# ActiveVisionLab/CrossScore

Measured on AMD Instinct MI355X. Metric: query-images/sec at 518x518, 5 ref views, bs=8; score-map MAE vs ref, higher is better.
Workload: dtype fp16

## Files before the change

### crossscore_amd/build.py

```python
from __future__ import annotations

import os
import subprocess
import sys

HERE = os.path.dirname(os.path.abspath(__file__))
CSRC = os.path.join(HERE, "csrc")
LIB = os.path.join(HERE, "libcrossscore_hip.so")
SOURCES = ["api.hip", "gemm.hip", "gemm256.hip", "attention.hip", "elementwise.hip", "preprocess.hip", "panel.hip", "panel4.hip", "patch.hip", "rowln.hip"]


EXTRA_FLAGS = {"panel.hip": ["-fno-slp-vectorize"], "panel4.hip": ["-fno-slp-vectorize"]}


def _hipcc() -> str:
    for c in (os.environ.get("HIPCC"), "/opt/rocm/bin/hipcc", "hipcc"):
        if c and (os.path.isabs(c) and os.path.exists(c) or not os.path.isabs(c)):
            return c
    return "hipcc"


def needs_build() -> bool:
    if not os.path.exists(LIB):
        return True
    t = os.path.getmtime(LIB)
    deps = [os.path.join(CSRC, f) for f in os.listdir(CSRC)] + [os.path.join(os.path.dirname(HERE), "include", "crossscore_hip.h")]
    return any(os.path.getmtime(d) > t for d in deps)


def build(force: bool = False, verbose: bool = True) -> str:
    if not force and not needs_build():
        return LIB
    objs = []
    procs = []
    os.makedirs(os.path.join(HERE, "build"), exist_ok=True)
    for s in SOURCES:
        o = os.path.join(HERE, "build", s.replace(".hip", ".o"))
        objs.append(o)
        cmd = [_hipcc(), "--offload-arch=gfx950", "-O3", "-std=c++17", "-fPIC", "-Wno-unused-value"] + EXTRA_FLAGS.get(s, []) + ["-c", os.path.join(CSRC, s), "-o", o]
        procs.append((cmd, subprocess.Popen(cmd, stdout=subprocess.PIPE, stderr=subprocess.STDOUT, text=True)))
    for cmd, p in procs:
        out, _ = p.communicate()
        if p.returncode != 0:
            raise RuntimeError("hipcc failed: " + " ".join(cmd) + "\n" + out)
        if verbose and out.strip():
            print(out, file=sys.stderr)
    cmd = [_hipcc(), "--offload-arch=gfx950", "-shared", "-fPIC", "-o", LIB] + objs
    r = subprocess.run(cmd, stdout=subprocess.PIPE, stderr=subprocess.STDOUT, text=True)
    if r.returncode != 0:
        raise RuntimeError("link failed: " + r.stdout)
    return LIB


if __name__ == "__main__":
    print(build(force="--force" in sys.argv))
```

### crossscore_amd/csrc/attention.hip

```cpp
#include "cs_common.h"
#include <atomic>
#include <math.h>

#ifdef CS_ATTN_STAMP
__device__ unsigned long long g_attn_dbg[64 * 4 * 8];
#define CS_TS(k) do { __builtin_amdgcn_sched_barrier(0); const unsigned long long now_ = __builtin_amdgcn_s_memtime(); \
    ph[k] += now_ - tlast; tlast = now_; __builtin_amdgcn_sched_barrier(0); } while (0)
#else
#define CS_TS(k) do { } while (0)
#endif

namespace {

template <int DH>
struct AttnCfg {
  static constexpr int KS = DH / 16;
  static constexpr int DT = (DH + 31) / 32;
  static constexpr int CH = DH / 8;
  static constexpr int KROW = DH * 2 + 16;
  static constexpr int VROW = (DH <= 16) ? 64 : (DH <= 96 ? 192 : (DH <= 128 ? 320 : 448));
  static_assert(VROW >= DT * 64 && (VROW / 4) % 32 == 16, "V row pitch");
  static constexpr int KTILE = 64 * KROW;
  static constexpr int VTILE = 64 * VROW;
  static constexpr int STAGE = KTILE + VTILE;
  static constexpr int NIT = (64 * CH + 255) / 256;
};

template <int DH, bool BF>
__global__ __launch_bounds__(256, DH > 128 ? 1 : 2) void cs_attn_kernel(CsAttnParams p) {
  using Cfg = AttnCfg<DH>;
  constexpr int KS = Cfg::KS, DT = Cfg::DT, CH = Cfg::CH, NIT = Cfg::NIT;
  extern __shared__ __attribute__((aligned(16))) char smem[];
  const int tid = threadIdx.x;
  const int lane = tid & 63;
  const int wv = __builtin_amdgcn_readfirstlane(tid >> 6);
  const int r = lane & 31;
  const int hh = lane >> 5;
  const int QB = (p.Lq + 127) / 128;
  const int xcd = blockIdx.x & 7, jj = blockIdx.x >> 3;
  const int gi = jj / QB, qb = jj - gi * QB;
  const int grp = gi * 8 + xcd;
  if (grp >= p.heads * p.nbatch) return;
  const int head = grp % p.heads;
  const int bat = grp / p.heads;
  const int q0 = qb * 128 + wv * 32;

  const h16_t* Qb = p.Q + (size_t)bat * p.q_bs + head * DH;
  const h16_t* Kb = p.K + (size_t)bat * p.k_bs + head * DH;
  const h16_t* Vb = p.V + (size_t)bat * p.v_bs + head * DH;

  h16x8_t qf[KS];
  {
    int qr = q0 + r;
    qr = qr < p.Lq ? qr : p.Lq - 1;
    const h16_t* qp = Qb + (size_t)qr * p.ldq + 8 * hh;
#pragma unroll
    for (int s = 0; s < KS; ++s) qf[s] = *reinterpret_cast<const h16x8_t*>(qp + 16 * s);
  }

  constexpr bool kFullLast = (64 * CH) % 256 == 0;
  int skey[NIT], sch[NIT];
#pragma unroll
  for (int it = 0; it < NIT; ++it) {
    const int c = tid + it * 256;
    skey[it] = c / CH;
    sch[it] = c - skey[it] * CH;
  }
  uint4 kreg[NIT], vreg[NIT];
#pragma unroll
  for (int it = 0; it < NIT; ++it) { kreg[it] = make_uint4(0, 0, 0, 0); vreg[it] = make_uint4(0, 0, 0, 0); }
  unsigned kgo[NIT], vgo[NIT];
#pragma unroll
  for (int it = 0; it < NIT; ++it) {
    kgo[it] = ((unsigned)skey[it] * (unsigned)p.ldk + (unsigned)sch[it] * 8u) * 2u;
    vgo[it] = ((unsigned)skey[it] * (unsigned)p.ldv + (unsigned)sch[it] * 8u) * 2u;
  }
  const unsigned k_bytes = (unsigned)(((size_t)(p.Lk - 1) * p.ldk + DH) * 2), v_bytes = (unsigned)(((size_t)(p.Lk - 1) * p.ldv + DH) * 2);
#define CS_ATTN_LOAD_TILE(T)                                                                       \
  {                                                                                                \
    const unsigned ks_ = (unsigned)(T) * 64u * (unsigned)p.ldk * 2u, vs_ = (unsigned)(T) * 64u * (unsigned)p.ldv * 2u; \
    const __amdgpu_buffer_rsrc_t k_rs = __builtin_amdgcn_make_buffer_rsrc(                         \
        const_cast<char*>(reinterpret_cast<const char*>(Kb)) + ks_, 0, (int)(k_bytes - ks_), 0x00020000); \
    const __amdgpu_buffer_rsrc_t v_rs = __builtin_amdgcn_make_buffer_rsrc(                         \
        const_cast<char*>(reinterpret_cast<const char*>(Vb)) + vs_, 0, (int)(v_bytes - vs_), 0x00020000); \
    _Pragma("unroll") for (int it = 0; it < NIT; ++it) {                                           \
      if (kFullLast || it + 1 < NIT || tid + it * 256 < 64 * CH) {                                 \
        kreg[it] = __builtin_bit_cast(uint4, __builtin_amdgcn_raw_buffer_load_b128(k_rs, kgo[it], 0, 0)); \
        vreg[it] = __builtin_bit_cast(uint4, __builtin_amdgcn_raw_buffer_load_b128(v_rs, vgo[it], 0, 0)); \
      }                                                                                            \
    }                                                                                              \
  }
#define CS_ATTN_WRITE_TILE(BUF)                                                                    \
  _Pragma("unroll") for (int it = 0; it < NIT; ++it) {                                             \
    if (kFullLast || it + 1 < NIT || tid + it * 256 < 64 * CH) {                                   \
      char* kb_ = smem + (BUF) * Cfg::STAGE;                                                       \
      *reinterpret_cast<uint4*>(kb_ + skey[it] * Cfg::KROW + sch[it] * 16) = kreg[it];             \
      *reinterpret_cast<uint4*>(kb_ + Cfg::KTILE + skey[it] * Cfg::VROW + sch[it] * 16) = vreg[it]; \
    }                                                                                              \
  }

  f32x16_t ot[DT];
#pragma unroll
  for (int d = 0; d < DT; ++d)
#pragma unroll
    for (int e = 0; e < 16; ++e) ot[d][e] = 0.f;
  constexpr float kTau = 8.0f;
  float m_run = 0.f;
  float l_run = 0.f;
  f32x16_t negm;
#pragma unroll
  for (int e = 0; e < 16; ++e) negm[e] = 0.f;
  {
    const float sc = p.scale_log2e;
    if (sc != 1.0f) {
#pragma unroll
      for (int s = 0; s < KS; ++s)
#pragma unroll
        for (int j = 0; j < 8; ++j) {
          const _Float16 e = qf[s][j];
          qf[s][j] = __builtin_bit_cast(_Float16, f2o<BF>(o2f<BF>(__builtin_bit_cast(h16_t, e)) * sc));
        }
    }
  }

  const int koff = r * Cfg::KROW + hh * 16;
  const int li = lane & 15, lg = (lane >> 4) & 1;
  const int voff = (4 * hh + (li >> 2)) * Cfg::VROW + (16 * lg + 4 * (li & 3)) * 2;

  const int nt = (p.Lk + 63) / 64;
  CS_ATTN_LOAD_TILE(0)
  CS_ATTN_WRITE_TILE(0)
  __syncthreads();
#ifdef CS_ATTN_STAMP
  unsigned long long ph[5] = {0, 0, 0, 0, 0};
  const unsigned long long tbegin = __builtin_amdgcn_s_memtime(), rbegin = __builtin_amdgcn_s_memrealtime();
  unsigned long long tlast = tbegin;
#endif
  for (int t = 0; t < nt; ++t) {
    if (t + 1 < nt) { CS_ATTN_LOAD_TILE(t + 1) }
    const char* kb = smem + (t & 1) * Cfg::STAGE;
    const char* vb = kb + Cfg::KTILE;

    f32x16_t st[2];
    float ps0 = 0.f, ps1 = 0.f;
    h16x8_t pf[2][2];
    auto scores = [&]() {
#pragma unroll
      for (int k2 = 0; k2 < 2; ++k2) {
#pragma unroll
        for (int s = 0; s < KS; ++s) {
          h16x8_t kf = *reinterpret_cast<const h16x8_t*>(kb + koff + k2 * 32 * Cfg::KROW + s * 32);
          st[k2] = mfma_32x32x16<BF>(kf, qf[s], s == 0 ? negm : st[k2]);
        }
      }
      if (t == nt - 1 && (p.Lk & 63)) {
        const int kbase = t * 64 + 4 * hh;
#pragma unroll
        for (int k2 = 0; k2 < 2; ++k2)
#pragma unroll
          for (int e = 0; e < 16; ++e) {
            const int key = kbase + k2 * 32 + (e & 3) + 8 * (e >> 2);
            if (key >= p.Lk) st[k2][e] = -INFINITY;
          }
      }
    };
    auto row_max = [&]() {
      float tm = st[0][0];
#pragma unroll
      for (int e = 1; e < 16; ++e) tm = fmaxf(tm, st[0][e]);
#pragma unroll
      for (int e = 0; e < 16; ++e) tm = fmaxf(tm, st[1][e]);
      return fmaxf(tm, __shfl_xor(tm, 32, 64));
    };
    auto move_reference = [&](float delta, bool first) {
      const float alpha = first ? 1.0f : __builtin_amdgcn_exp2f(-delta);
      m_run += delta;
#pragma unroll
      for (int e = 0; e < 16; ++e) negm[e] = -m_run;
      asm volatile("" : "+v"(negm));
#pragma unroll
      for (int k2 = 0; k2 < 2; ++k2)
#pragma unroll
        for (int e = 0; e < 16; ++e) st[k2][e] -= delta;
      l_run *= alpha;
#pragma unroll
      for (int d = 0; d < DT; ++d)
#pragma unroll
        for (int e = 0; e < 16; ++e) ot[d][e] *= alpha;
    };
    auto exp_pack = [&]() {
      ps0 = 0.f; ps1 = 0.f;
#pragma unroll
      for (int k2 = 0; k2 < 2; ++k2)
#pragma unroll
        for (int s2 = 0; s2 < 2; ++s2) {
#pragma unroll
          for (int j = 0; j < 8; j += 2) {
            const float pa = __builtin_amdgcn_exp2f(st[k2][8 * s2 + j]);
            const float pb = __builtin_amdgcn_exp2f(st[k2][8 * s2 + j + 1]);
            ps0 += pa;
            ps1 += pb;
            pf[k2][s2][j] = __builtin_bit_cast(_Float16, f2o<BF>(pa));
            pf[k2][s2][j + 1] = __builtin_bit_cast(_Float16, f2o<BF>(pb));
          }
        }
    };
    scores();
    const float tmax = row_max();
    CS_TS(0);
    if (t == 0 || __builtin_amdgcn_ballot_w64(tmax > kTau) != 0) move_reference(t == 0 ? tmax : fmaxf(tmax, 0.f), t == 0);
    exp_pack();
    l_run += ps0 + ps1;
    CS_TS(1);

#pragma unroll
    for (int k2 = 0; k2 < 2; ++k2)
#pragma unroll
      for (int s2 = 0; s2 < 2; ++s2) {
        const char* vrow = vb + voff + (k2 * 32 + 16 * s2) * Cfg::VROW;
#pragma unroll
        for (int d = 0; d < DT; ++d) {
          short4_t lo = __builtin_amdgcn_ds_read_tr16_b64_v4i16(
              (__attribute__((address_space(3))) short4_t*)(vrow + d * 64));
          short4_t hi = __builtin_amdgcn_ds_read_tr16_b64_v4i16(
              (__attribute__((address_space(3))) short4_t*)(vrow + 8 * Cfg::VROW + d * 64));
          short8_t vf8 = __builtin_shufflevector(lo, hi, 0, 1, 2, 3, 4, 5, 6, 7);
          ot[d] = mfma_32x32x16<BF>(__builtin_bit_cast(h16x8_t, vf8), pf[k2][s2], ot[d]);
        }
      }

    CS_TS(2);
    if (t + 1 < nt) { CS_ATTN_WRITE_TILE((t + 1) & 1) }
    CS_TS(3);
    __syncthreads();
    CS_TS(4);
  }
#ifdef CS_ATTN_STAMP
  if (blockIdx.x % 50 == 0 && blockIdx.x / 50 < 64 && lane == 0) {
    unsigned long long* d = g_attn_dbg + (blockIdx.x / 50 * 4 + wv) * 8;
    for (int k = 0; k < 5; ++k) d[k] = ph[k];
    d[5] = rbegin;
    d[6] = __builtin_amdgcn_s_memtime() - tbegin;
    d[7] = __builtin_amdgcn_s_memrealtime() - rbegin;
  }
#endif

  const float l_tot = l_run + __shfl_xor(l_run, 32, 64);
  const float inv = 1.0f / l_tot;
  const int q = q0 + r;
  if (q < p.Lq) {
    h16_t* op = p.O + (size_t)bat * p.o_bs + (size_t)q * p.ldo + head * DH;
#pragma unroll
    for (int d = 0; d < DT; ++d)
#pragma unroll
      for (int g4 = 0; g4 < 4; ++g4) {
        const int dd = d * 32 + 8 * g4 + 4 * hh;
        if (dd < DH) {
          const float v0 = ot[d][4 * g4 + 0] * inv, v1 = ot[d][4 * g4 + 1] * inv, v2 = ot[d][4 * g4 + 2] * inv, v3 = ot[d][4 * g4 + 3] * inv;
          uint2 o;
          o.x = pack_o16x2<BF>(v0, v1);
          o.y = pack_o16x2<BF>(v2, v3);
          *reinterpret_cast<uint2*>(op + dd) = o;
        }
      }
    if (p.lse && hh == 0) p.lse[((size_t)bat * p.heads + head) * p.Lq + q] = m_run + log2f(l_tot);
  }
}

template <int DH, bool BF>
hipError_t launch(CsAttnParams p, int batch, hipStream_t stream) {
  p.nbatch = batch;
  const int groups = p.heads * batch;
  dim3 grid(((groups + 7) / 8) * 8 * ((p.Lq + 127) / 128));
  const int lds = 2 * AttnCfg<DH>::STAGE + 64;
  if (lds > 48 * 1024) {
    static std::atomic<bool> attr_done[16];
    int dev = 0;
    if (hipGetDevice(&dev) != hipSuccess || dev < 0 || dev >= 16) return hipErrorInvalidDevice;
    if (!attr_done[dev]) {
      hipError_t e = hipFuncSetAttribute(reinterpret_cast<const void*>(cs_attn_kernel<DH, BF>), hipFuncAttributeMaxDynamicSharedMemorySize, lds);
      if (e != hipSuccess) return e;
      attr_done[dev] = true;
    }
  }
  hipLaunchKernelGGL((cs_attn_kernel<DH, BF>), grid, dim3(256), lds, stream, p);
  return hipGetLastError();
}

}

#ifdef CS_ATTN_STAMP
extern "C" int cs_attn_debug_read(unsigned long long* dst) { return (int)hipMemcpyFromSymbol(dst, HIP_SYMBOL(g_attn_dbg), sizeof(g_attn_dbg)); }
#endif

extern "C" const char* cs_attn_check(const CsAttnParams* p, int dh, int batch) {
  if (dh != 16 && dh != 48 && dh != 64 && dh != 96 && dh != 128 && dh != 192) return "attention: head dim must be 16, 48, 64, 96, 128 or 192";
  if (p->Lq <= 0 || p->Lk <= 0 || p->heads <= 0 || batch <= 0) return "attention: empty shape";
  if ((long long)batch * p->heads * ((p->Lq + 127) / 128) > (1ll << 30)) return "attention: grid too large";
  if (p->ldq % 8 || p->ldk % 8 || p->ldv % 8 || p->ldo % 4) return "attention: row strides must keep 16-byte rows";
  if (p->q_bs % 8 || p->k_bs % 8 || p->v_bs % 8 || p->o_bs % 4) return "attention: batch strides must keep 16-byte rows";
  if (!p->Q || !p->K || !p->V || !p->O) return "attention: null operand";
  if ((long long)p->Lk * p->ldk >= (1ll << 30) || (long long)p->Lk * p->ldv >= (1ll << 30)) return "attention: Lk * row stride must stay below 2^30 elements (32-bit tile offsets)";
  return nullptr;
}

extern "C" hipError_t cs_attn_launch(const CsAttnParams* p, int dh, int batch, hipStream_t stream) {
  switch (dh) {
    case 16: return p->bf16 ? launch<16, true>(*p, batch, stream) : launch<16, false>(*p, batch, stream);
    case 48: return p->bf16 ? launch<48, true>(*p, batch, stream) : launch<48, false>(*p, batch, stream);
    case 64: return p->bf16 ? launch<64, true>(*p, batch, stream) : launch<64, false>(*p, batch, stream);
    case 96: return p->bf16 ? launch<96, true>(*p, batch, stream) : launch<96, false>(*p, batch, stream);
    case 128: return p->bf16 ? launch<128, true>(*p, batch, stream) : launch<128, false>(*p, batch, stream);
    case 192: return p->bf16 ? launch<192, true>(*p, batch, stream) : launch<192, false>(*p, batch, stream);
  }
  return hipErrorInvalidValue;
}
```

Before: 1325.

## Add 16x16x32 MFMA attention path for head dims 48/64 with full/tail tile split

For head dims 48 and 64, the attention kernel now uses 16x16x32 MFMA tiles with two 16-row query sub-tiles per wave. It also uses tighter K/V LDS row pitches, which lets the launch bound allow 3 blocks per CU. This removes the padding waste the 32x32 tiles incurred at small head dims and cuts LDS footprint. Both the new path and the generic path now specialise full tiles versus the ragged last tile, skip dead query waves and half-empty key blocks, and compile with SLP vectorisation off. The risks are more code, higher register pressure from two accumulator sets, and possible correctness issues in the masking/zero-padding for DH=48.

```diff
diff --git a/crossscore_amd/build.py b/crossscore_amd/build.py
--- a/crossscore_amd/build.py
+++ b/crossscore_amd/build.py
@@ -10,7 +10,7 @@
 SOURCES = ["api.hip", "gemm.hip", "gemm256.hip", "attention.hip", "elementwise.hip", "preprocess.hip", "panel.hip", "panel4.hip", "patch.hip", "rowln.hip"]
 
 
-EXTRA_FLAGS = {"panel.hip": ["-fno-slp-vectorize"], "panel4.hip": ["-fno-slp-vectorize"]}
+EXTRA_FLAGS = {"panel.hip": ["-fno-slp-vectorize"], "panel4.hip": ["-fno-slp-vectorize"], "attention.hip": ["-fno-slp-vectorize"]}
 
 
 def _hipcc() -> str:
diff --git a/crossscore_amd/csrc/attention.hip b/crossscore_amd/csrc/attention.hip
--- a/crossscore_amd/csrc/attention.hip
+++ b/crossscore_amd/csrc/attention.hip
@@ -1,6 +1,7 @@
 #include "cs_common.h"
 #include <atomic>
 #include <math.h>
+#include <type_traits>
 
 #ifdef CS_ATTN_STAMP
 __device__ unsigned long long g_attn_dbg[64 * 4 * 8];
@@ -14,12 +15,16 @@
 
 template <int DH>
 struct AttnCfg {
+  static constexpr bool T16 = DH == 48 || DH == 64;
   static constexpr int KS = DH / 16;
   static constexpr int DT = (DH + 31) / 32;
+  static constexpr int KS2 = (DH + 31) / 32;
+  static constexpr int DT16 = DH / 16;
   static constexpr int CH = DH / 8;
-  static constexpr int KROW = DH * 2 + 16;
-  static constexpr int VROW = (DH <= 16) ? 64 : (DH <= 96 ? 192 : (DH <= 128 ? 320 : 448));
-  static_assert(VROW >= DT * 64 && (VROW / 4) % 32 == 16, "V row pitch");
+  static constexpr int KROW = T16 ? 160 : DH * 2 + 16;
+  static constexpr int VROW = T16 ? (DH == 64 ? 160 : 96) : (DH <= 16) ? 64 : (DH <= 96 ? 192 : (DH <= 128 ? 320 : 448));
+  static_assert(T16 ? (VROW >= DH * 2 && (VROW / 4) % 16 == 8 && KROW >= KS2 * 64 && (KROW / 16) % 4 == 2)
+                    : (VROW >= DT * 64 && (VROW / 4) % 32 == 16), "K / V row pitch");
   static constexpr int KTILE = 64 * KROW;
   static constexpr int VTILE = 64 * VROW;
   static constexpr int STAGE = KTILE + VTILE;
@@ -27,7 +32,7 @@
 };
 
 template <int DH, bool BF>
-__global__ __launch_bounds__(256, DH > 128 ? 1 : 2) void cs_attn_kernel(CsAttnParams p) {
+__global__ __launch_bounds__(256, DH > 128 ? 1 : (AttnCfg<DH>::T16 ? 3 : 2)) void cs_attn_kernel(CsAttnParams p) {
   using Cfg = AttnCfg<DH>;
   constexpr int KS = Cfg::KS, DT = Cfg::DT, CH = Cfg::CH, NIT = Cfg::NIT;
   extern __shared__ __attribute__((aligned(16))) char smem[];
@@ -49,15 +54,6 @@
   const h16_t* Kb = p.K + (size_t)bat * p.k_bs + head * DH;
   const h16_t* Vb = p.V + (size_t)bat * p.v_bs + head * DH;
 
-  h16x8_t qf[KS];
-  {
-    int qr = q0 + r;
-    qr = qr < p.Lq ? qr : p.Lq - 1;
-    const h16_t* qp = Qb + (size_t)qr * p.ldq + 8 * hh;
-#pragma unroll
-    for (int s = 0; s < KS; ++s) qf[s] = *reinterpret_cast<const h16x8_t*>(qp + 16 * s);
-  }
-
   constexpr bool kFullLast = (64 * CH) % 256 == 0;
   int skey[NIT], sch[NIT];
 #pragma unroll
@@ -99,6 +95,227 @@
     }                                                                                              \
   }
 
+  if constexpr (Cfg::T16) {
+    constexpr int KS2 = Cfg::KS2, DT16 = Cfg::DT16;
+    const int li = lane & 15, g = lane >> 4;
+    const int nqt = __builtin_amdgcn_readfirstlane(q0 >= p.Lq ? 0 : (q0 + 16 >= p.Lq ? 1 : 2));
+    if constexpr (DH == 48) {
+      const int zrow = (tid >> 1) & 63;
+      *reinterpret_cast<uint4*>(smem + (tid >> 7) * Cfg::STAGE + zrow * Cfg::KROW + 96 + 16 * (tid & 1)) = make_uint4(0, 0, 0, 0);
+    }
+    h16x8_t qf[2][KS2];
+#pragma unroll
+    for (int qt = 0; qt < 2; ++qt) {
+      int qr = q0 + 16 * qt + li;
+      qr = qr < p.Lq ? qr : p.Lq - 1;
+      const h16_t* qp = Qb + (size_t)qr * p.ldq + 8 * g;
+#pragma unroll
+      for (int s = 0; s < KS2; ++s) {
+#pragma unroll
+        for (int j = 0; j < 8; ++j) qf[qt][s][j] = (_Float16)0.f;
+        if (32 * s + 32 <= DH || 32 * s + 8 * g < DH) qf[qt][s] = *reinterpret_cast<const h16x8_t*>(qp + 32 * s);
+      }
+    }
+    {
+      const float sc = p.scale_log2e;
+      if (sc != 1.0f) {
+#pragma unroll
+        for (int qt = 0; qt < 2; ++qt)
+#pragma unroll
+          for (int s = 0; s < KS2; ++s)
+#pragma unroll
+            for (int j = 0; j < 8; ++j) {
+              const _Float16 e = qf[qt][s][j];
+              qf[qt][s][j] = __builtin_bit_cast(_Float16, f2o<BF>(o2f<BF>(__builtin_bit_cast(h16_t, e)) * sc));
+            }
+      }
+    }
+    f32x4_t ot[2][DT16];
+#pragma unroll
+    for (int qt = 0; qt < 2; ++qt)
+#pragma unroll
+      for (int d = 0; d < DT16; ++d)
+#pragma unroll
+        for (int e = 0; e < 4; ++e) ot[qt][d][e] = 0.f;
+    constexpr float kTau = 8.0f;
+    float m_run[2] = {0.f, 0.f};
+    float l_run[2] = {0.f, 0.f};
+    f32x4_t negm[2];
+#pragma unroll
+    for (int qt = 0; qt < 2; ++qt)
+#pragma unroll
+      for (int e = 0; e < 4; ++e) negm[qt][e] = 0.f;
+
+    const int koff = li * Cfg::KROW + g * 16;
+    const int voff = (4 * g + (li >> 2)) * Cfg::VROW + (li & 3) * 8;
+
+    const int nt = (p.Lk + 63) / 64;
+    CS_ATTN_LOAD_TILE(0)
+    CS_ATTN_WRITE_TILE(0)
+    __syncthreads();
+#ifdef CS_ATTN_STAMP
+    unsigned long long ph[5] = {0, 0, 0, 0, 0};
+    const unsigned long long tbegin = __builtin_amdgcn_s_memtime(), rbegin = __builtin_amdgcn_s_memrealtime();
+    unsigned long long tlast = tbegin;
+#endif
+    auto tile = [&](auto full_c, const int t, const int nkt) __attribute__((always_inline)) {
+      constexpr bool FULL = decltype(full_c)::value;
+      const char* kb = smem + (t & 1) * Cfg::STAGE;
+      const char* vb = kb + Cfg::KTILE;
+      f32x4_t st[2][4];
+      h16x8_t pf[2][2];
+      float tm[2] = {-INFINITY, -INFINITY};
+#pragma unroll
+      for (int kt = 0; kt < 4; ++kt) {
+        if (FULL || kt < nkt) {
+          if (!FULL) __builtin_amdgcn_sched_barrier(0);
+#pragma unroll
+          for (int s = 0; s < KS2; ++s) {
+            const h16x8_t kf = *reinterpret_cast<const h16x8_t*>(kb + koff + kt * 16 * Cfg::KROW + s * 64);
+#pragma unroll
+            for (int qt = 0; qt < 2; ++qt)
+              if (FULL || qt < nqt) st[qt][kt] = mfma_16x16x32<BF>(kf, qf[qt][s], s == 0 ? negm[qt] : st[qt][kt]);
+          }
+#pragma unroll
+          for (int qt = 0; qt < 2; ++qt)
+            if (FULL || qt < nqt) {
+              if (!FULL) {
+                const int key = t * 64 + kt * 16 + 4 * g;
+#pragma unroll
+                for (int j = 0; j < 4; ++j)
+                  if (key + j >= p.Lk) st[qt][kt][j] = -INFINITY;
+              }
+#pragma unroll
+              for (int j = 0; j < 4; ++j) tm[qt] = fmaxf(tm[qt], st[qt][kt][j]);
+            }
+        }
+      }
+      CS_TS(0);
+      if (t == 0 || __builtin_amdgcn_ballot_w64(fmaxf(tm[0], tm[1]) > kTau) != 0) {
+#pragma unroll
+        for (int qt = 0; qt < 2; ++qt)
+          if (FULL || qt < nqt) {
+            float rm = fmaxf(tm[qt], __shfl_xor(tm[qt], 16, 64));
+            rm = fmaxf(rm, __shfl_xor(rm, 32, 64));
+            const float delta = t == 0 ? rm : fmaxf(rm, 0.f);
+            const float alpha = t == 0 ? 1.0f : __builtin_amdgcn_exp2f(-delta);
+            m_run[qt] += delta;
+#pragma unroll
+            for (int e = 0; e < 4; ++e) negm[qt][e] = -m_run[qt];
+            asm volatile("" : "+v"(negm[qt]));
+#pragma unroll
+            for (int kt = 0; kt < 4; ++kt)
+              if (FULL || kt < nkt)
+#pragma unroll
+                for (int j = 0; j < 4; ++j) st[qt][kt][j] -= delta;
+            l_run[qt] *= alpha;
+#pragma unroll
+            for (int d = 0; d < DT16; ++d)
+#pragma unroll
+              for (int e = 0; e < 4; ++e) ot[qt][d][e] *= alpha;
+          }
+      }
+      if (!FULL) __builtin_amdgcn_sched_barrier(0);
+#pragma unroll
+      for (int qt = 0; qt < 2; ++qt)
+        if (FULL || qt < nqt) {
+          float ps0 = 0.f, ps1 = 0.f;
+#pragma unroll
+          for (int kt = 0; kt < 4; ++kt) {
+            if (FULL || kt < nkt) {
+#pragma unroll
+              for (int j = 0; j < 4; j += 2) {
+                const float pa = __builtin_amdgcn_exp2f(st[qt][kt][j]);
+                const float pb = __builtin_amdgcn_exp2f(st[qt][kt][j + 1]);
+                ps0 += pa;
+                ps1 += pb;
+                pf[qt][kt >> 1][4 * (kt & 1) + j] = __builtin_bit_cast(_Float16, f2o<BF>(pa));
+                pf[qt][kt >> 1][4 * (kt & 1) + j + 1] = __builtin_bit_cast(_Float16, f2o<BF>(pb));
+              }
+            } else {
+#pragma unroll
+              for (int j = 0; j < 4; ++j) pf[qt][kt >> 1][4 * (kt & 1) + j] = (_Float16)0.f;
+            }
+          }
+          l_run[qt] += ps0 + ps1;
+        }
+      CS_TS(1);
+      if (!FULL) __builtin_amdgcn_sched_barrier(0);
+#pragma unroll
+      for (int s = 0; s < 2; ++s)
+        if (FULL || 2 * s < nkt) {
+          const char* vrow = vb + voff + 32 * s * Cfg::VROW;
+#pragma unroll
+          for (int d = 0; d < DT16; ++d) {
+            short4_t lo = __builtin_amdgcn_ds_read_tr16_b64_v4i16(
+                (__attribute__((address_space(3))) short4_t*)(vrow + d * 32));
+            short4_t hi = __builtin_amdgcn_ds_read_tr16_b64_v4i16(
+                (__attribute__((address_space(3))) short4_t*)(vrow + 16 * Cfg::VROW + d * 32));
+            const short8_t vf8 = __builtin_shufflevector(lo, hi, 0, 1, 2, 3, 4, 5, 6, 7);
+#pragma unroll
+            for (int qt = 0; qt < 2; ++qt)
+              if (FULL || qt < nqt) ot[qt][d] = mfma_16x16x32<BF>(__builtin_bit_cast(h16x8_t, vf8), pf[qt][s], ot[qt][d]);
+          }
+        }
+      CS_TS(2);
+    };
+    auto run = [&](auto full_c, const int t0, const int t1) __attribute__((always_inline)) {
+      for (int t = t0; t < t1; ++t) {
+        if (t + 1 < nt) { CS_ATTN_LOAD_TILE(t + 1) }
+        if (decltype(full_c)::value || nqt > 0) {
+          const int left = p.Lk - t * 64;
+          tile(full_c, t, left >= 64 ? 4 : (left + 15) >> 4);
+        }
+        if (t + 1 < nt) { CS_ATTN_WRITE_TILE((t + 1) & 1) }
+        CS_TS(3);
+        __syncthreads();
+        CS_TS(4);
+      }
+    };
+    const int ntf = nqt == 2 ? ((p.Lk & 63) ? nt - 1 : nt) : 0;
+    run(std::true_type{}, 0, ntf);
+    run(std::false_type{}, ntf, nt);
+#ifdef CS_ATTN_STAMP
+    if (blockIdx.x % 50 == 0 && blockIdx.x / 50 < 64 && lane == 0) {
+      unsigned long long* d = g_attn_dbg + (blockIdx.x / 50 * 4 + wv) * 8;
+      for (int k = 0; k < 5; ++k) d[k] = ph[k];
+      d[5] = rbegin;
+      d[6] = __builtin_amdgcn_s_memtime() - tbegin;
+      d[7] = __builtin_amdgcn_s_memrealtime() - rbegin;
+    }
+#endif
+
+    const int le = __builtin_amdgcn_mbcnt_hi(~0u, __builtin_amdgcn_mbcnt_lo(~0u, 0u));
+    const int lie = le & 15, ge = le >> 4;
+#pragma unroll
+    for (int qt = 0; qt < 2; ++qt) {
+      float l_tot = l_run[qt] + __shfl_xor(l_run[qt], 16, 64);
+      l_tot += __shfl_xor(l_tot, 32, 64);
+      const float inv = 1.0f / l_tot;
+      const int q = q0 + 16 * qt + lie;
+      if (q < p.Lq) {
+        h16_t* op = p.O + (size_t)bat * p.o_bs + (size_t)q * p.ldo + head * DH + 4 * ge;
+#pragma unroll
+        for (int d = 0; d < DT16; ++d) {
+          uint2 o;
+          o.x = pack_o16x2<BF>(ot[qt][d][0] * inv, ot[qt][d][1] * inv);
+          o.y = pack_o16x2<BF>(ot[qt][d][2] * inv, ot[qt][d][3] * inv);
+          *reinterpret_cast<uint2*>(op + 16 * d) = o;
+        }
+        if (p.lse && ge == 0) p.lse[((size_t)bat * p.heads + head) * p.Lq + q] = m_run[qt] + log2f(l_tot);
+      }
+    }
+  } else
+  {
+  h16x8_t qf[KS];
+  {
+    int qr = q0 + r;
+    qr = qr < p.Lq ? qr : p.Lq - 1;
+    const h16_t* qp = Qb + (size_t)qr * p.ldq + 8 * hh;
+#pragma unroll
+    for (int s = 0; s < KS; ++s) qf[s] = *reinterpret_cast<const h16x8_t*>(qp + 16 * s);
+  }
+
   f32x16_t ot[DT];
 #pragma unroll
   for (int d = 0; d < DT; ++d)
@@ -136,8 +353,10 @@
   const unsigned long long tbegin = __builtin_amdgcn_s_memtime(), rbegin = __builtin_amdgcn_s_memrealtime();
   unsigned long long tlast = tbegin;
 #endif
-  for (int t = 0; t < nt; ++t) {
-    if (t + 1 < nt) { CS_ATTN_LOAD_TILE(t + 1) }
+  const bool live_w = q0 < p.Lq;
+  auto tile = [&](auto last_c, const int t) __attribute__((always_inline)) {
+    constexpr bool LAST = decltype(last_c)::value;
+    const bool two = !LAST || p.Lk - t * 64 > 32;
     const char* kb = smem + (t & 1) * Cfg::STAGE;
     const char* vb = kb + Cfg::KTILE;
 
@@ -147,13 +366,18 @@
     auto scores = [&]() {
 #pragma unroll
       for (int k2 = 0; k2 < 2; ++k2) {
-#pragma unroll
-        for (int s = 0; s < KS; ++s) {
-          h16x8_t kf = *reinterpret_cast<const h16x8_t*>(kb + koff + k2 * 32 * Cfg::KROW + s * 32);
-          st[k2] = mfma_32x32x16<BF>(kf, qf[s], s == 0 ? negm : st[k2]);
-        }
-      }
-      if (t == nt - 1 && (p.Lk & 63)) {
+        if (k2 == 0 || two) {
+#pragma unroll
+          for (int s = 0; s < KS; ++s) {
+            h16x8_t kf = *reinterpret_cast<const h16x8_t*>(kb + koff + k2 * 32 * Cfg::KROW + s * 32);
+            st[k2] = mfma_32x32x16<BF>(kf, qf[s], s == 0 ? negm : st[k2]);
+          }
+        } else {
+#pragma unroll
+          for (int e = 0; e < 16; ++e) st[k2][e] = -INFINITY;
+        }
+      }
+      if (LAST && (p.Lk & 63)) {
         const int kbase = t * 64 + 4 * hh;
 #pragma unroll
         for (int k2 = 0; k2 < 2; ++k2)
@@ -194,6 +418,7 @@
       for (int k2 = 0; k2 < 2; ++k2)
 #pragma unroll
         for (int s2 = 0; s2 < 2; ++s2) {
+          if (k2 == 1 && !two) continue;
 #pragma unroll
           for (int j = 0; j < 8; j += 2) {
             const float pa = __builtin_amdgcn_exp2f(st[k2][8 * s2 + j]);
@@ -217,6 +442,7 @@
     for (int k2 = 0; k2 < 2; ++k2)
 #pragma unroll
       for (int s2 = 0; s2 < 2; ++s2) {
+        if (k2 == 1 && !two) continue;
         const char* vrow = vb + voff + (k2 * 32 + 16 * s2) * Cfg::VROW;
 #pragma unroll
         for (int d = 0; d < DT; ++d) {
@@ -230,11 +456,19 @@
       }
 
     CS_TS(2);
-    if (t + 1 < nt) { CS_ATTN_WRITE_TILE((t + 1) & 1) }
-    CS_TS(3);
-    __syncthreads();
-    CS_TS(4);
-  }
+  };
+  auto run = [&](auto last_c, const int t0, const int t1) __attribute__((always_inline)) {
+    for (int t = t0; t < t1; ++t) {
+      if (t + 1 < nt) { CS_ATTN_LOAD_TILE(t + 1) }
+      if (live_w) tile(last_c, t);
+      if (t + 1 < nt) { CS_ATTN_WRITE_TILE((t + 1) & 1) }
+      CS_TS(3);
+      __syncthreads();
+      CS_TS(4);
+    }
+  };
+  run(std::false_type{}, 0, nt - 1);
+  run(std::true_type{}, nt - 1, nt);
 #ifdef CS_ATTN_STAMP
   if (blockIdx.x % 50 == 0 && blockIdx.x / 50 < 64 && lane == 0) {
     unsigned long long* d = g_attn_dbg + (blockIdx.x / 50 * 4 + wv) * 8;
@@ -264,6 +498,7 @@
         }
       }
     if (p.lse && hh == 0) p.lse[((size_t)bat * p.heads + head) * p.Lq + q] = m_run + log2f(l_tot);
+  }
   }
 }
 
```

Result: faster. 1353, median of 6 (+2.1%).
